# jepsen-io/maelstrom

Hardware: NVIDIA H100
Metric: simulated msgs/sec (broadcast, 4096 nodes) (higher is better)
Workload: dtype int64

## Files before the change

### maelstrom_b200/csrc/ms_device.cuh

```cuda
#pragma once
#include <stdint.h>
#include "../../include/maelstrom_b200.h"

#if defined(__CUDACC__)
#define MS_HD __host__ __device__ __forceinline__
#else
#define MS_HD inline
#endif

namespace msd {

constexpr int64_t  kTickNs   = 1000000;
constexpr uint32_t kInjector = 0xFFFFFFFFu;
constexpr uint8_t  kRemoved  = 0x80;

enum : uint32_t {
  E_NONE = 0, E_RING_OVERFLOW = 1, E_WINDOW_OVERFLOW = 2, E_JOURNAL_OVERFLOW = 3,
  E_INVALID_DEST = 4, E_HISTORY = 5, E_VALUE_RANGE = 6, E_MAIL_OVERFLOW = 7,
  E_CALENDAR_OVERFLOW = 8, E_ID_RANGE = 9, E_BARRIER = 10, E_SNAPSHOT = 11,
  E_RAFT_CAPACITY = 12, E_HISTORY_RING = 13
};

#ifndef MS_CLS0_NT
#define MS_CLS0_NT 64
// ... 132 lines not shown
  uint32_t* gs_tag;
  uint32_t* gs_snap;
  uint32_t  gs_slots, gs_interval_ms;
  uint32_t  family;
  uint32_t  sv_ep[4];
  uint32_t  sv_n_keys;
  uint32_t* sv_lin_val;
  uint8_t*  sv_lin_has;
  uint32_t* sv_lww_val;
  uint8_t*  sv_lww_has;
  uint64_t* sv_scalars;
  uint32_t* sv_seq_cli;
  uint32_t* sv_seq_vidx;
  uint32_t* sv_seq_vval;
  uint8_t*  sv_seq_vhas;
  uint32_t* sv_seq_vcnt;
  uint32_t* gs_snap_sh[8];
  uint32_t* gs_tag_sh[8];
  struct RaftDev* rf_node;
  uint4*    rf_log;
  uint32_t* rf_kv_val;
  uint8_t*  rf_kv_has;
  int32_t*  rf_next;
  int32_t*  rf_match;
  int32_t*  rf_scratch;
  uint4*    rf_cb;
  uint32_t* rf_votes;
  uint4*    rf_stage;
  uint4*    rf_heap;
  unsigned long long* rf_heap_cursor;
  uint64_t* rf_ext_off;
  uint32_t* rf_ext_tag;
  uint32_t  rf_log_cap, rf_n_keys, rf_stage_cap, rf_heap_mask, rf_vote_words;
  uint32_t  rf_group;
  uint32_t  rf_gmax;
  uint32_t  rf_cb_mask;
  struct TreeDev* tt_node;
  unsigned char* tt_recs;
  uint32_t* tt_cache;
  uint4*    tt_queue;
  uint32_t  tt_per_node, tt_cache_mask;
  struct GenDev* gc;
  uint4*    gc_hist;
  uint32_t  gc_hist_mask, gc_n, gc_read_permille, gc_pad;
  int64_t   gc_interval_ns, gc_timeout_ns, gc_limit_ns, gc_quiet_ns;
  uint4*    rf_heap_sh[8];
  uint64_t* rf_ext_off_sh[8];
  uint32_t* rf_ext_tag_sh[8];
  uint32_t  kv_value_range, kv_keys_per_group;
  int64_t   kv_key_period_ns;
  struct NemDev* nem;
  uint32_t  nem_clusters, nem_group, nem_targets, nem_pad;
  int64_t   nem_interval_ns, nem_limit_ns;
};

constexpr uint32_t kRaftCallbacks = 4096;
constexpr uint32_t kRaftExt = 1024;
constexpr int64_t  kElectionTimeoutNs = 2000000000;
constexpr int64_t  kHeartbeatNs = 1000000000;
constexpr int64_t  kMinReplicationNs = 50000000;
enum : int32_t { RAFT_NASCENT = 0, RAFT_FOLLOWER = 1, RAFT_CANDIDATE = 2, RAFT_LEADER = 3 };

struct RaftDev {
  int32_t  state;
  uint32_t term;
  int32_t  voted_for, leader;
  uint32_t commit_index, last_applied;
  int64_t  election_deadline, step_down_deadline, last_replication;
  uint32_t next_msg_id, log_size, appends, n_votes, kv_size;
  uint32_t busy;
};

constexpr uint32_t kTreeQueue = 256;
struct TreeDev {
  uint32_t ptr_counter;
  uint32_t phase;
  uint32_t cur_src, cur_msg_id;
  uint64_t cur_ops;
  uint32_t root1, root2, start_counter, writes_left, write_failed, load_ptr;
  uint32_t q_head, q_tail;
  uint32_t init_src, init_msg_id;
  uint32_t init_phase;
  uint32_t gen;
  uint32_t first_write, first_write_ok, root_is_leaf;
  uint32_t pad;
  int64_t  deadline, init_deadline;
};
constexpr int64_t kPromiseTimeoutNs = 5000000000ll;

struct GenDev {
  uint32_t next_msg_id, waiting_for;
  int64_t  deadline_ns;
  int64_t  next_op_ns;
  uint32_t node;
  uint32_t ops;
  union { uint32_t bcasts;
          uint32_t key_base; };
  uint32_t phase;
  uint32_t cur_f, cur_value;
  uint32_t ordinal;
  uint32_t reader;
};
enum : uint32_t { GEN_MIX = 0, GEN_QUIET = 1, GEN_FINAL = 2, GEN_DONE = 3 };

constexpr uint32_t kSeqBuffer = 32;
constexpr uint32_t kSeqHist = kSeqBuffer + 1;
// ... 19 lines not shown
MS_HD uint64_t mulhi64(uint64_t a, uint64_t b) {
#if defined(__CUDA_ARCH__)
  return __umul64hi(a, b);
#else
  return (uint64_t)(((unsigned __int128)a * b) >> 64);
#endif
}

MS_HD int clz64(uint64_t x) {
#if defined(__CUDA_ARCH__)
  return __clzll((long long)x);
#else
  return __builtin_clzll(x);
#endif
}

MS_HD uint64_t neg_log2_q32(uint64_t X) {
  if (X == ~0ull) return 0;
  const uint64_t Y = X + 1;
  const int n = 63 - clz64(Y);
  uint64_t m = Y << (63 - n);
  uint32_t frac = 0;
  for (int i = 31; i >= 0; i--) {
    const uint64_t hi = mulhi64(m, m);
    if (hi >> 63) { frac |= (1u << i); m = hi; }
    else          { m = hi << 1; }
  }
  return (64ull << 32) - (((uint64_t)n << 32) | frac);
}

MS_HD uint64_t latency_ms(const NetParams& np, const uint32_t x[4]) {
  if (np.dist == MS_DIST_CONSTANT) return (uint64_t)np.mean_ms * np.scale;
  if (np.dist == MS_DIST_UNIFORM)
    return (((uint64_t)x[1] * (2ull * np.mean_ms)) >> 32) * np.scale;
  const uint64_t X = ((uint64_t)x[2] << 32) | x[1];
  return mulhi64(neg_log2_q32(X), np.exp_coeff);
}

MS_HD bool kind_is_client(uint8_t k) { k &= 0x7F; return k == MS_KIND_CLIENT || k == MS_KIND_SIM_CLIENT || k == MS_KIND_GEN_CLIENT; }

MS_HD uint32_t owner_of(uint32_t e, uint32_t n_servers, uint32_t G) {
  if (G <= 1) return 0;
  if (e < n_servers) return (uint32_t)(((uint64_t)e * G) / n_servers);
  return (e - n_servers) % G;
}
MS_HD uint32_t owner_of_ticket(uint32_t t, uint32_t n_inj, uint32_t n_servers, uint32_t G) {
  return t < n_inj ? 0u : owner_of(t - n_inj, n_servers, G);
}

MS_HD uint64_t compact_round(uint64_t round, uint32_t round_lo) {
  return round - (uint32_t)((uint32_t)round - round_lo);
}

}
```

### maelstrom_b200/csrc/ms_engine.cu

```cuda
#include <cuda_runtime.h>
#include <math.h>
#include <stdio.h>
#include <stdlib.h>
#include <string.h>

#include <algorithm>
#include <deque>
#include <mutex>
#include <new>
#include <string>
#include <unordered_map>
#include <vector>

#include "ms_device.cuh"
#include "ms_nemesis.h"
#include "ms_tree.h"
#include "ms_fressian.h"
#include "ms_json.h"

using namespace msd;

extern "C" {
cudaError_t msk_round_smem_attr(size_t bytes);
size_t msk_round_smem_bytes(uint32_t cap);
// ... 541 lines not shown
  c.server_max_window = c.server_max_window ? pow2_at_least(c.server_max_window) : std::min(c.max_window, c.server_ring_cap);
  if (c.server_max_window > c.server_ring_cap) c.server_max_window = c.server_ring_cap;
  if (c.server_max_window > c.max_window) {
    set_err("server_max_window must not exceed max_window");
    return MS_ERR_ARG;
  }
  if (!c.journal_cap_log2) c.journal_cap_log2 = 22;
  if (c.journal_level > 2) c.journal_level = 2;
  if (!c.mailbox_cap) c.mailbox_cap = 1u << 16;
  if (!c.inject_cap) c.inject_cap = 1u << 16;
  if (!c.gset_interval_ms) c.gset_interval_ms = 5000;
  s->use_calendar = c.latency_mean_ms > 0;
  if (s->use_calendar) {
    c.calendar_slots = pow2_at_least(c.calendar_slots ? c.calendar_slots
                                                      : std::min<uint32_t>(16384u, std::max<uint32_t>(64u, 32u * c.latency_mean_ms)));
    const uint32_t hist = history_rows(c.reserved[0], c.max_endpoints + 8u);
    while (c.calendar_slots > 4 && c.calendar_slots > hist / 4) c.calendar_slots >>= 1;
    if (!c.calendar_cap) c.calendar_cap = 1u << 16;
  }
  if (c.n_shards == 0) c.n_shards = 1;
  if (c.n_shards > 8 || c.shard_id >= c.n_shards) { set_err("n_shards must be <= 8 and shard_id < n_shards"); return MS_ERR_ARG; }
  if (c.threads_per_node && (c.threads_per_node % 32 || c.threads_per_node > 512)) {
    set_err("threads_per_node must be a multiple of 32 in [32,512]");
    return MS_ERR_ARG;
  }
  {
    const uint32_t* ladder = kClsLadder;
    const int thr_gset[4] = {256, 256, 256, 512};
    const int* thr = c.workload == MS_W_GSET ? thr_gset : kClsThreads;
    s->n_classes = 0;
    for (int k = 0; k < 4; k++) {
      const uint32_t cap = std::min(ladder[k], c.max_window);
      s->class_cap[s->n_classes] = cap;
      s->class_threads[s->n_classes] = c.threads_per_node ? (int)c.threads_per_node : thr[k];
      s->n_classes++;
      if (cap == c.max_window) break;
    }
  }

  int ndev = 0;
  if (cudaGetDeviceCount(&ndev) != cudaSuccess || ndev == 0) {
    set_err("no CUDA device: maelstrom_b200 has no CPU fallback");
    return MS_ERR_CUDA;
  }
  s->device = c.device;
  CK(cudaSetDevice(s->device));
  CK(cudaStreamCreateWithFlags(&s->stream, cudaStreamNonBlocking));
  for (int k = 0; k < 4; k++) CK(cudaStreamCreateWithFlags(&s->aux_streams[k], cudaStreamNonBlocking));
  for (int k = 0; k < 5; k++) CK(cudaEventCreateWithFlags(&s->aux_events[k], cudaEventDisableTiming));

  Params& P = s->P;
  memset(&P, 0, sizeof P);
  const uint32_t M = c.max_endpoints;
  const bool compact = c.workload == MS_W_BROADCAST;
  const size_t n_ctr = (size_t)M + (compact ? c.n_nodes : 0u);
  int rc;
  if ((rc = s->dalloc(&P.st, 1))) return rc;
  if ((rc = s->dalloc(&P.np, 1))) return rc;
  if ((rc = s->dalloc(&P.kind, M))) return rc;
  if ((rc = s->dalloc(&P.tail, n_ctr))) return rc;
  if ((rc = s->dalloc(&P.limit, n_ctr))) return rc;
  if ((rc = s->dalloc(&P.head, n_ctr))) return rc;
  if ((rc = s->dalloc(&P.ep_born, M))) return rc;
  {
    const size_t full_vecs = ((size_t)c.n_nodes * c.server_ring_cap + (size_t)(M - c.n_nodes) * c.ring_cap) * 3;
    const size_t compact_vecs = compact ? (size_t)c.n_nodes * c.server_ring_cap : 0;
    void* ptr = nullptr;
    CK(cudaMalloc(&ptr, (full_vecs + compact_vecs) * 16));
    s->allocs.push_back(ptr);
    P.ring = (uint4*)ptr;
    P.cring_off = full_vecs;
    P.cq = compact ? M : 0u;
  }
  P.ring_cap = c.ring_cap;
  P.ring_cap_s = c.server_ring_cap;
  P.n_servers = c.n_nodes;
  P.n_ep = c.n_nodes;
  P.n_inj_tickets = 8;
  P.max_window = c.max_window;
  P.max_window_s = c.server_max_window;
  s->use_graph = c.reserved[1] == 1;
  P.n_shards = c.n_shards;
  P.shard_id = c.shard_id;
  {
    P.t_max = M + P.n_inj_tickets;
    const uint32_t hist = history_rows(c.reserved[0], P.t_max);
    P.hist = hist;
    P.hist_mask = hist - 1;
    if ((rc = s->dalloc(&P.rmeta, hist))) return rc;
    if ((rc = s->dalloc(&P.rt_em, (size_t)hist * P.t_max))) return rc;
    if ((rc = s->dalloc(&P.rt_ev, (size_t)hist * P.t_max))) return rc;
    if ((rc = s->dalloc(&P.rt_chunk, (size_t)hist * P.t_max))) return rc;
    if ((rc = s->dalloc(&P.rt_cnt, (size_t)hist * P.t_max))) return rc;
    std::vector<RoundMeta> init(hist);
    memset(init.data(), 0, init.size() * sizeof(RoundMeta));
    for (uint32_t i = 1; i < hist; i++) init[i].round = ~0ull;
    CK(cudaMemcpyAsync(P.rmeta, init.data(), init.size() * sizeof(RoundMeta), cudaMemcpyHostToDevice, s->stream));
    CK(cudaStreamSynchronize(s->stream));
  }
  P.jlevel = c.journal_level;
  P.jdiscard = c.journal_discard;
  if (c.journal_level) {
    const uint64_t J = 1ull << c.journal_cap_log2;
    void* ptr = nullptr;
    CK(cudaMalloc(&ptr, J * 16));
    s->allocs.push_back(ptr);
    P.jraw = (uint4*)ptr;
    P.jmask = J - 1;
    if (c.journal_level >= 2) {
      CK(cudaMalloc(&ptr, J * 32));
      s->allocs.push_back(ptr);
      P.jbody = (uint4*)ptr;
    }
  }
  if ((rc = s->dalloc(&P.comp, M))) return rc;
  P.seed_lo = c.seed_lo;
  P.seed_hi = c.seed_hi;
  P.workload = c.workload;
  P.topology = c.topology;
  P.n_values = c.n_values;
  P.bm_words = (c.n_values + 31) / 32;
  if (c.workload == MS_W_BROADCAST || c.workload == MS_W_GSET) {
    if ((rc = s->dalloc(&P.bitmap, (size_t)c.n_nodes * P.bm_words))) return rc;
    if ((rc = s->dalloc(&P.set_count, c.n_nodes))) return rc;
    if (c.topology != MS_TOPO_TOTAL) {
      std::vector<uint32_t> off(c.n_nodes + 1, 0), nbr, tmp;
      for (uint32_t k = 0; k < c.n_nodes; k++) {
        topo_neighbors(c.topology, c.n_nodes, k, tmp);
        nbr.insert(nbr.end(), tmp.begin(), tmp.end());
        off[k + 1] = (uint32_t)nbr.size();
      }
      if ((rc = s->dalloc(&P.nbr_off, off.size()))) return rc;
      if ((rc = s->dalloc(&P.nbr, nbr.size() + 1))) return rc;
      CK(cudaMemcpyAsync(P.nbr_off, off.data(), off.size() * 4, cudaMemcpyHostToDevice, s->stream));
      if (!nbr.empty()) CK(cudaMemcpyAsync(P.nbr, nbr.data(), nbr.size() * 4, cudaMemcpyHostToDevice, s->stream));
      CK(cudaStreamSynchronize(s->stream));
    }
  } else if (c.workload == MS_W_ECHO) {
    if ((rc = s->dalloc(&P.next_msg_id, c.n_nodes))) return rc;
  }
  P.family = c.workload == MS_W_GSET ? 1u : (c.workload >= MS_W_RAFT ? 4u : 0u);
  if (c.workload == MS_W_TXN_TREE) {
    if (c.n_shards > 1) { set_err("MS_W_TXN_TREE runs on one GPU (tree records are read across nodes)"); return MS_ERR_ARG; }
    const size_t N = c.n_nodes;
    P.tt_per_node = c.reserved[3] ? c.reserved[3] : 256u;
    P.tt_cache_mask = pow2_at_least(c.reserved[4] ? c.reserved[4] : 1024u) - 1u;
    const uint64_t n_ptrs = 2ull + (uint64_t)N * P.tt_per_node;
    if (n_ptrs > (1ull << 31)) { set_err("MS_W_TXN_TREE: n_nodes x reserved[3] pointers do not fit"); return MS_ERR_ARG; }
    if (!c.reserved[2]) c.reserved[2] = (uint32_t)n_ptrs;
    if ((rc = s->dalloc(&P.tt_node, N)) || (rc = s->dalloc(&P.tt_recs, (size_t)n_ptrs * 64)) ||
        (rc = s->dalloc(&P.tt_cache, N * ((size_t)P.tt_cache_mask + 1))) || (rc = s->dalloc(&P.tt_queue, N * kTreeQueue)))
      return rc;
    mst::Rec empty{};
    empty.type = 1; empty.lo = 0; empty.hi = (uint8_t)mst::kRing; empty.n = 0;
    CK(cudaMemcpyAsync(P.tt_recs + (size_t)(mst::kPtrEmpty - 1u) * 64, &empty, sizeof empty, cudaMemcpyHostToDevice, s->stream));
    CK(cudaStreamSynchronize(s->stream));
  }
  if (c.workload == MS_W_TXN || c.workload == MS_W_TXN_TREE) {
    const size_t N = c.n_nodes;
    P.rf_stage_cap = c.workload == MS_W_TXN_TREE ? c.server_max_window * (mst::kMaxWrites + 2u) + 64u : c.server_max_window + 16u;
    P.rf_cb_mask = pow2_at_least(c.reserved[5] ? c.reserved[5] : kRaftCallbacks) - 1u;
    if (c.workload == MS_W_TXN_TREE && P.rf_cb_mask + 1u < 128u) P.rf_cb_mask = 127u;
    if ((rc = s->dalloc(&P.rf_node, N)) || (rc = s->dalloc(&P.rf_cb, N * ((size_t)P.rf_cb_mask + 1) * 2)) ||
        (rc = s->dalloc(&P.rf_stage, N * P.rf_stage_cap * 3)))
      return rc;
  }
  if (c.workload == MS_W_RAFT) {
    const size_t N = c.n_nodes;
    P.rf_n_keys = c.reserved[2] ? c.reserved[2] : 4096u;
    P.rf_log_cap = c.reserved[3] ? c.reserved[3] : 4096u;
    P.rf_group = (c.reserved[4] && c.reserved[4] < c.n_nodes) ? c.reserved[4] : 0u;
    P.rf_gmax = P.rf_group ? P.rf_group : c.n_nodes;
    P.rf_cb_mask = pow2_at_least(c.reserved[5] ? c.reserved[5] : kRaftCallbacks) - 1u;
    P.rf_stage_cap = c.server_max_window + 2u * P.rf_gmax + P.rf_log_cap + 16u;
    P.rf_vote_words = (P.rf_gmax + 31u) / 32u;
    const uint64_t heap_want = std::max<uint64_t>(std::max<uint64_t>(1u << 16, 8ull * P.rf_log_cap), 64ull * c.n_nodes);
    if (heap_want > (1ull << 30)) { set_err("Raft payload heap too large"); return MS_ERR_ARG; }
    const uint32_t heap_words = pow2_at_least((uint32_t)heap_want);
    P.rf_heap_mask = heap_words - 1u;
    if ((rc = s->dalloc(&P.rf_node, N)) || (rc = s->dalloc(&P.rf_log, N * P.rf_log_cap * 2)) ||
        (rc = s->dalloc(&P.rf_kv_val, N * P.rf_n_keys)) || (rc = s->dalloc(&P.rf_kv_has, N * P.rf_n_keys)) ||
        (rc = s->dalloc(&P.rf_next, N * P.rf_gmax)) || (rc = s->dalloc(&P.rf_match, N * P.rf_gmax)) ||
        (rc = s->dalloc(&P.rf_scratch, N * P.rf_gmax)) || (rc = s->dalloc(&P.rf_cb, N * ((size_t)P.rf_cb_mask + 1) * 2)) ||
        (rc = s->dalloc(&P.rf_votes, N * P.rf_vote_words)) || (rc = s->dalloc(&P.rf_stage, N * P.rf_stage_cap * 3)) ||
        (rc = s->dalloc(&P.rf_heap, (size_t)heap_words)) || (rc = s->dalloc(&P.rf_heap_cursor, 1)) ||
        (rc = s->dalloc(&P.rf_ext_off, N * kRaftExt + (N * kRaftExt + 1) / 2)))
      return rc;
    P.rf_ext_tag = reinterpret_cast<uint32_t*>(P.rf_ext_off + N * kRaftExt);
// ... 1421 lines not shown
```

### maelstrom_b200/csrc/ms_kernels.cu

```cuda
#include <cuda_runtime.h>
#include <stdint.h>
#include "ms_device.cuh"
#include "ms_nemesis.h"

namespace msd {

#define FULL 0xFFFFFFFFu
#ifndef MS_EMUL
#define MS_LAUNCH(kern, grid, block, smem, stream, ...) kern<<<(grid), (block), (smem), (stream)>>>(__VA_ARGS__)
#endif
constexpr int MAXB = 64;
constexpr int MAXNB = 8;
constexpr uint64_t RECV_BIT = 1ull << 63;
constexpr uint32_t kResolvedTicket = 0xFFFFFFu;

__device__ __forceinline__ void st_v4(uint4* p, uint4 v) {
#ifdef MS_EMUL
  *p = v;
#else
  asm volatile("st.global.L1::no_allocate.v4.u32 [%0], {%1,%2,%3,%4};" ::"l"(p), "r"(v.x), "r"(v.y),
               "r"(v.z), "r"(v.w)
               : "memory");
#endif
}
// ... 17 lines not shown
  (void)gptr; (void)bytes;
#endif
}

__device__ __forceinline__ void latch_error(DevState* st, uint32_t code, uint32_t arg) {
  if (atomicCAS(&st->error, 0u, code) == 0u) st->error_arg = arg;
}

__device__ __forceinline__ bool round_skipped(const Params& p, const DevState* st) {
  if (st->now >= st->stop_ns || st->error) return true;
  if (p.jlevel && !p.jdiscard) {
    const uint64_t raw_base = p.rmeta[(uint32_t)st->round & p.hist_mask].raw_base;
    if (p.n_shards <= 1 && raw_base - st->jraw_drained > ((p.jmask + 1) >> 1)) return true;
    if (st->round - st->drain_round + 2 >= p.hist) return true;
  }
  return false;
}

__device__ __forceinline__ uint32_t slot_tag(uint64_t round) { return 0x80000000u | (uint32_t)(round & 0x7FFFFFFFull); }

struct Rec {
  uint64_t round;
  uint32_t ticket, idx;
  uint32_t src, dest, msg_id, in_reply_to;
  uint32_t tf;
  uint32_t p0;
  uint64_t p1;
};

__device__ __forceinline__ void rec_store(uint4* slot, const Rec& r) {
  st_v4(slot + 0, make_uint4(r.idx, r.ticket, (uint32_t)r.round, (uint32_t)(r.round >> 32)));
  st_v4(slot + 1, make_uint4(r.src, r.dest, r.msg_id, r.in_reply_to));
  st_v4(slot + 2, make_uint4(r.tf, r.p0, (uint32_t)r.p1, (uint32_t)(r.p1 >> 32)));
}
__device__ __forceinline__ Rec rec_unpack(uint4 a, uint4 b, uint4 c) {
  Rec r;
  r.idx = a.x; r.ticket = a.y;
  r.round = (uint64_t)a.z | ((uint64_t)a.w << 32);
  r.src = b.x; r.dest = b.y; r.msg_id = b.z; r.in_reply_to = b.w;
  r.tf = c.x; r.p0 = c.y;
  r.p1 = (uint64_t)c.z | ((uint64_t)c.w << 32);
  return r;
}

__device__ __forceinline__ uint32_t ring_cap_of(const Params& p, uint32_t e) { return e < p.n_servers ? p.ring_cap_s : p.ring_cap; }
__device__ __forceinline__ size_t ring_base(const Params& p, uint32_t e) {
  return e < p.n_servers ? (size_t)e * p.ring_cap_s
                         : (size_t)p.n_servers * p.ring_cap_s + (size_t)(e - p.n_servers) * p.ring_cap;
}
__device__ __forceinline__ uint4* ring_slot(const Params& p, uint4* ring, uint32_t e, uint32_t pos) {
  return ring + (ring_base(p, e) + (pos & (ring_cap_of(p, e) - 1u))) * 3;
}

__device__ __forceinline__ uint4* cring_slot(const Params& p, uint4* ring, uint32_t e, uint32_t pos) {
  return ring + p.cring_off + (size_t)e * p.ring_cap_s + (pos & (p.ring_cap_s - 1u));
}

struct Win {
  const uint4* ring;
  const uint4* cring;
  uint32_t head, chead, mask, n_full;
};
__device__ __forceinline__ void win_load(const Params& p, const Win& w, uint32_t e, uint64_t round, uint32_t i,
                                         uint4& a, uint4& b, uint4& c) {
  if (i < w.n_full) {
    const uint4* rp = w.ring + (size_t)((w.head + i) & w.mask) * 3;
    a = rp[0]; b = rp[1]; c = rp[2];
  } else {
    const uint4 x = w.cring[(w.chead + (i - w.n_full)) & w.mask];
    a = make_uint4(x.x, x.y, x.z, (uint32_t)(compact_round(round, x.z) >> 32));
    b = make_uint4(x.y - p.n_inj_tickets, e, 0u, 0u);
    c = make_uint4((uint32_t)MS_T_BROADCAST, x.w, 0u, 0u);
  }
}
__device__ __forceinline__ Rec win_rec(const Params& p, const Win& w, uint32_t e, uint64_t round, uint32_t i) {
  uint4 a, b, c;
  win_load(p, w, e, round, i, a, b, c);
  return rec_unpack(a, b, c);
}

struct RoundSmem {
  uint64_t* reg1;
  uint32_t* keyB;
  uint32_t* vals;
  uint16_t* tab;
  uint16_t* meta;
  uint16_t* ord;
  uint8_t* blk;
};

__device__ __forceinline__ uint64_t dense_base(const Params& p, DevState* st, uint64_t round, uint32_t ticket) {
  if (ticket == kResolvedTicket) return round << 32;
  const uint32_t row = (uint32_t)round & p.hist_mask;
  const RoundMeta* m = p.rmeta + row;
  if (m->round != round || ticket >= p.t_max) {
    latch_error(st, E_HISTORY, (uint32_t)round);
    return 0;
  }
  return m->id_base + p.rt_em[(size_t)row * p.t_max + ticket];
}

__device__ __forceinline__ uint64_t cta_excl_scan_u64(uint64_t sum, int nt, int lane, int warp, uint64_t* wtmp ) {
  uint64_t incl = sum;
#pragma unroll
  for (int d = 1; d < 32; d <<= 1) {
    const uint64_t y = __shfl_up_sync(FULL, incl, d);
    if (lane >= d) incl += y;
  }
  if (lane == 31) wtmp[warp] = incl;
  __syncthreads();
  if (warp == 0) {
    const int nw = nt >> 5;
    const uint64_t w = lane < nw ? wtmp[lane] : 0;
    uint64_t wi = w;
#pragma unroll
    for (int d = 1; d < 32; d <<= 1) {
      const uint64_t y = __shfl_up_sync(FULL, wi, d);
      if (lane >= d) wi += y;
    }
    wtmp[lane] = wi - w;
    if (lane == 31) wtmp[32] = wi;
  }
  __syncthreads();
  return wtmp[warp] + incl - sum;
}
// ... 1268 lines not shown
    if (cdirty) { p.sv_lin_has[ck] = chas ? 1 : 0; p.sv_lin_val[ck] = cval; }
  }
  __syncthreads();
}

#ifndef MS_ROUND_MINB2
#define MS_ROUND_MINB2 4
#endif
template <int CLS> struct ClsShape {
  static constexpr uint32_t cap = kClsLadder[CLS < 3 ? CLS : 2];
  static constexpr int nt = kClsThreads[CLS];
};

template <int CLS, int WL, bool FIX = false>
__global__ void __launch_bounds__(CLS == 3 ? 512 : 256, CLS == 3 ? 2 : MS_ROUND_MINB2) k_round(Params p, uint32_t cap_arg) {
  constexpr uint32_t cls = CLS;
  static_assert(!FIX || CLS < 3, "class 3 is sized by max_window");
  const uint32_t cap = FIX ? ClsShape<CLS>::cap : cap_arg;
  constexpr bool GS = (WL & 1) != 0;
  constexpr bool SV = (WL & 2) != 0;
  constexpr bool RF = (WL & 4) != 0;
  DevState* st = p.st;

#ifdef MS_EMUL
  unsigned char* smem_raw = simt::dyn_smem();
#else
  extern __shared__ __align__(16) unsigned char smem_raw[];
#endif
  uint64_t* reg1 = reinterpret_cast<uint64_t*>(smem_raw);
  uint32_t* keyB = reinterpret_cast<uint32_t*>(reg1 + cap + 1);
  uint32_t* vals = keyB + cap;
  uint16_t* tab = reinterpret_cast<uint16_t*>(vals + cap);
  uint16_t* meta = tab + 2 * (size_t)cap;
  uint16_t* ord = meta + cap;
  uint8_t* blk = reinterpret_cast<uint8_t*>(ord + cap);
  const RoundSmem sm{reg1, keyB, vals, tab, meta, ord, blk};
  uint64_t* keyA = reg1;
  uint64_t* aux = reg1;

  __shared__ uint64_t s_wtmp[34];
  __shared__ NetParams s_np;
  __shared__ uint32_t s_wcnt[17];
  __shared__ uint32_t s_misc[8];
  __shared__ uint32_t s_cnt[8];
  __shared__ uint64_t s_chunk;
  __shared__ uint16_t s_bstart[MAXB + 1];
  __shared__ uint16_t s_brank[MAXB];
  __shared__ uint16_t s_boff[MAXB + 1];
  __shared__ uint64_t s_bkeyA[MAXB];
  __shared__ uint64_t s_bbase[MAXB];
  __shared__ uint16_t s_S[MAXB + 1][MAXNB];
  __shared__ uint32_t s_nbbase[MAXNB];
  __shared__ uint32_t s_nbr[MAXNB];
  __shared__ uint4 s_gen[2];
  __shared__ uint64_t s_round0;
  __shared__ int64_t s_now0;
  __shared__ uint32_t s_go;

  const int tid = threadIdx.x, nt = FIX ? ClsShape<CLS>::nt : (int)blockDim.x, lane = tid & 31;
  if (tid == 0) {
    s_np = *p.np;
    const uint32_t so = ld_volatile_u32(&st->slot_open);
    __threadfence();
    const uint64_t r = *reinterpret_cast<const volatile uint64_t*>(&st->round);
    s_round0 = r;
    s_now0 = *reinterpret_cast<const volatile int64_t*>(&st->now);
    s_go = (so == slot_tag(r) && !round_skipped(p, st)) ? 1u : 0u;
  }
  __syncthreads();
  if (!s_go) return;
  const NetParams np = s_np;
  const int64_t now = s_now0;
  const uint64_t round = s_round0;
  const uint32_t T = p.n_inj_tickets + p.n_ep;
  const uint32_t row = (uint32_t)round & p.hist_mask;
  const uint32_t par = (uint32_t)round & 1u;
  const uint32_t my_big = st->cls_count[par][cls];
  const uint32_t my_count = my_big + st->cls_small[par][cls];
  const uint32_t* my_list = p.cls_list + ((size_t)par * 4 + cls) * p.t_max;
  const uint32_t tag = ((uint32_t)round & 0x7FFFu) + 1u;
  const bool need_rng = np.loss_thresh != 0 || np.dist != MS_DIST_CONSTANT;
  const uint64_t const_lat = (uint64_t)np.mean_ms * np.scale;
#ifdef MS_PHASE_TIMING
  const bool timing = p.phase_cycles != nullptr;
#else
  constexpr bool timing = false;
#endif
  long long t_prev = timing ? clock64() : 0;
#define PHASE_MARK(k)                                                                         \
  do {                                                                                        \
    if (timing && tid == 0) {                                                                 \
      const long long t_now = clock64();                                                      \
      atomicAdd((unsigned long long*)&p.phase_cycles[cls * 16 + (k)], (unsigned long long)(t_now - t_prev)); \
      t_prev = t_now;                                                                         \
    }                                                                                         \
  } while (0)
  if (tid == 0) s_misc[5] = atomicAdd(&st->cls_cursor[par][cls], 1u);

 for (;;) {
  __syncthreads();
  const uint32_t li = s_misc[5];
  if (tid < 5) s_misc[tid] = 0;
  if (tid < 8) s_cnt[tid] = 0;
  __syncthreads();
  if (li >= my_count) break;
  uint32_t next_li = 0;
// ... 16 lines not shown
  uint32_t c_recv_cl = 0, c_replies = 0;
  uint32_t n_ev_local = 0, n_em_local = 0;

  if (ticket < p.n_inj_tickets) {
    const uint32_t n_host = st->inj_count;
    const uint64_t tick = (uint64_t)(now / kTickNs);
    const uint32_t cur = st->sched_cursor;
    uint32_t hi = (tick + 1 < p.n_tick_off) ? p.tick_off[tick + 1] : p.n_sched;
    if (hi < cur) hi = cur;
    const uint32_t K = n_host + (hi - cur);
    const uint32_t chunk = (K + p.n_inj_tickets - 1) / p.n_inj_tickets;
    const uint32_t lo = min(ticket * chunk, K), hi_s = min(lo + chunk, K);
    const uint32_t n_local = hi_s - lo;
    n_ev_local = n_local; n_em_local = n_local;
    if (tid == 0) journal_claim(p, st, n_local, ticket, s_chunk);
    __syncthreads();
    cx.chunk = s_chunk;
    cx.emitter = kInjector;
    cx.idx_bias = lo;
    for (uint32_t base = 0; base < n_local; base += nt) {
      const uint32_t j = base + tid;
      const bool valid = j < n_local;
      Rec r;
      r.dest = 0; r.src = 0;
      if (valid) {
        const uint32_t g = lo + j;
        if (g < n_host) {
          const ms_msg m = p.inj_buf[g];
          r.src = m.src; r.dest = m.dest; r.msg_id = m.msg_id; r.in_reply_to = m.in_reply_to;
          r.tf = (uint32_t)m.type | ((uint32_t)m.flags << 16); r.p0 = m.p0; r.p1 = m.p1;
        } else {
          const ms_op op = p.sched[cur + (g - n_host)];
          r.src = op.src; r.dest = op.dest; r.msg_id = op.body.msg_id; r.in_reply_to = op.body.in_reply_to;
          r.tf = (uint32_t)op.body.type | ((uint32_t)op.body.flags << 16); r.p0 = op.body.p0; r.p1 = op.body.p1;
        }
      }
      emit_one(p, st, np, cx, valid, r, j, 0, false);
    }
  } else {
    const uint32_t e = ticket - p.n_inj_tickets;
    const uint8_t kind = p.kind[e];
    const uint32_t head = p.head[e];
    const bool has_c = p.cq && e < p.n_servers;
    const uint32_t chead = has_c ? p.head[p.cq + e] : 0u;
    uint32_t n_full = p.limit[e] - head;
    uint32_t n = n_full + (has_c ? p.limit[p.cq + e] - chead : 0u);
    if (kind & kRemoved) n = n_full = 0;
    if (n > cap || n > (e < p.n_servers ? p.max_window_s : p.max_window)) {
      if (tid == 0) latch_error(st, E_WINDOW_OVERFLOW, e);
      n = n_full = 0;
    }
    const uint4* myring = p.ring + ring_base(p, e) * 3;
    const uint32_t my_mask = ring_cap_of(p, e) - 1u;
    const Win win{myring, p.ring + p.cring_off + (size_t)e * p.ring_cap_s, head, chead, my_mask, n_full};
    const bool is_server = (kind == MS_KIND_SERVER);
    const bool bcast = !GS && is_server && p.workload == MS_W_BROADCAST;
    uint32_t n_timer = 0, fire_seq = 0, fire_p0 = 0;
    if constexpr (GS) {
      if (is_server && p.gs_init[e] && now >= p.gs_next_fire[e]) {
        n_timer = p.n_servers - 1;
        fire_seq = p.gs_fires[e] + 1;
      }
    }
    const uint32_t* mybits = (is_server && p.bitmap) ? p.bitmap + (size_t)e * p.bm_words : nullptr;
    const uint32_t deg = bcast ? nbr_count(p, e) : 0;
    const bool nb_smem = bcast && p.topology != MS_TOPO_TOTAL && deg <= MAXNB;
    if (nb_smem && tid < (int)deg) s_nbr[tid] = p.nbr[p.nbr_off[e] + tid];
    __syncthreads();

    {
      uint32_t err_val = 0xFFFFFFFFu;
      uint32_t snap_gone = 0xFFFFFFFFu;
      bool inj_srv = false;
      const bool nb4 = nb_smem && deg <= 4;
      const uint32_t nr0 = (nb4 && deg > 0) ? s_nbr[0] : 0xFFFFFFFFu, nr1 = (nb4 && deg > 1) ? s_nbr[1] : 0xFFFFFFFFu;
      const uint32_t nr2 = (nb4 && deg > 2) ? s_nbr[2] : 0xFFFFFFFFu, nr3 = (nb4 && deg > 3) ? s_nbr[3] : 0xFFFFFFFFu;
      for (int base = 0; base < (int)n; base += 2 * nt) {
        uint4 a[2], b[2], c[2];
#pragma unroll
        for (int q = 0; q < 2; q++) {
          const int i = base + q * nt + tid;
          if (i < (int)n) win_load(p, win, e, round, (uint32_t)i, a[q], b[q], c[q]);
        }
#pragma unroll
        for (int q = 0; q < 2; q++) {
          const int i = base + q * nt + tid;
          if (i >= (int)n) continue;
          const uint64_t rnd = (uint64_t)a[q].z | ((uint64_t)a[q].w << 32);
          keyA[i] = (rnd << 24) | (uint64_t)(a[q].y & 0xFFFFFFu);
          keyB[i] = a[q].x;
          const uint32_t src = b[q].x, tf = c[q].x, v = c[q].y;
          if (a[q].y < p.n_inj_tickets && src < p.n_servers) inj_srv = true;
          bool cut = false;
          if (np.pair_active && p.pair_bits)
            cut = (p.pair_bits[(size_t)e * p.pair_words + (src >> 5)] >> (src & 31)) & 1u;
          if (!cut && np.comp_active) {
            const uint32_t cs = p.comp[src], ce = p.comp[e];
            cut = cs != ce && cs != 0xFFFFFFFFu && ce != 0xFFFFFFFFu;
          }
          const uint32_t type = tf & 0xFFFFu;
          const uint32_t fl = tf >> 16;
          uint32_t tc = TC_OTHER;
          if constexpr (GS) {
            if (type == MS_T_INIT) tc = GT_INIT;
            else if (type == MS_T_ADD) tc = GT_ADD;
            else if (type == MS_T_READ) tc = GT_READ;
            else if (type == MS_T_REPLICATE_ONE) tc = GT_REPL_ONE;
            else if (type == MS_T_REPLICATE_FULL) tc = GT_REPL_FULL;
          } else {
          if (type == MS_T_INIT) tc = TC_INIT;
          else if (type == MS_T_TOPOLOGY) tc = TC_TOPOLOGY;
          else if (type == MS_T_READ) tc = TC_READ;
          else if (type == MS_T_BROADCAST) tc = TC_BROADCAST;
          else if (type == MS_T_ECHO) tc = TC_ECHO;
          }
          uint32_t slot = 0;
          if (nb4) {
            slot = src == nr3 ? 4u : src == nr2 ? 3u : src == nr1 ? 2u : src == nr0 ? 1u : 0u;
          } else if (nb_smem) {
            for (uint32_t j = 0; j < deg; j++) if (s_nbr[j] == src) slot = j + 1;
// ... 10 lines not shown
          if constexpr (GS) {
            if (is_server && !cut && !(fl & MS_F_REPLY)) {
              if (tc == GT_ADD || tc == GT_REPL_ONE) {
                if (v >= p.n_values || v > V_MASK) err_val = v;
                else val |= v;
              } else if (tc == GT_REPL_FULL) {
                const uint32_t run = c[q].z;
                const uint32_t rowi = src * p.gs_slots + (run & (p.gs_slots - 1));
                if (src >= p.n_servers ||
                    __ldcg(p.gs_tag_sh[owner_of(src, p.n_servers, p.n_shards)] + rowi) != run) snap_gone = src;
                else val |= rowi;
              }
            }
          }
          vals[i] = val;
        }
      }
      if (err_val != 0xFFFFFFFFu) latch_error(st, E_VALUE_RANGE, err_val);
      if (snap_gone != 0xFFFFFFFFu) latch_error(st, E_SNAPSHOT, snap_gone);
      if (inj_srv) s_misc[3] = 1;
    }
    if (bcast) {
      for (int base = 0; base < (int)n; base += 4 * nt) {
        uint32_t w[4], vv[4];
#pragma unroll
        for (int q = 0; q < 4; q++) {
          const int i = base + q * nt + tid;
          vv[q] = i < (int)n ? vals[i] : 0u;
          w[q] = (vv[q] & V_CAND) ? mybits[(vv[q] & V_MASK) >> 5] : 0xFFFFFFFFu;
        }
#pragma unroll
        for (int q = 0; q < 4; q++) {
          const int i = base + q * nt + tid;
          if (i < (int)n && (vv[q] & V_CAND) && !((w[q] >> (vv[q] & 31)) & 1u)) vals[i] = vv[q] | V_FRESH;
        }
      }
    }
    __syncthreads();
    PHASE_MARK(1);
    if (tid == 0 && next_li < my_count) {
      const uint32_t t2 = list_ticket(my_list, my_big, p.t_max, next_li);
      if (t2 >= p.n_inj_tickets) {
        const uint32_t e2 = t2 - p.n_inj_tickets;
        const uint32_t h2 = p.head[e2], n2 = p.limit[e2] - h2, cap2 = ring_cap_of(p, e2);
        if (n2 > 0 && n2 <= cap2) {
          const uint4* base2 = p.ring + ring_base(p, e2) * 3;
          const uint32_t o2 = h2 & (cap2 - 1u), first = min(n2, cap2 - o2);
          prefetch_l2_bulk(base2 + (size_t)o2 * 3, first * 48u);
          if (n2 > first) prefetch_l2_bulk(base2, (n2 - first) * 48u);
        }
        if (p.cq && e2 < p.n_servers) {
          const uint32_t ch2 = p.head[p.cq + e2], nc2 = p.limit[p.cq + e2] - ch2;
          if (nc2 > 0 && nc2 <= cap2) {
            const uint4* cbase2 = p.ring + p.cring_off + (size_t)e2 * cap2;
            const uint32_t o2 = ch2 & (cap2 - 1u), first = min(nc2, cap2 - o2);
            prefetch_l2_bulk(cbase2 + o2, first * 16u);
            if (nc2 > first) prefetch_l2_bulk(cbase2, (nc2 - first) * 16u);
          }
        }
      }
    }

    uint32_t R = 0;
    bool use_blocks = false;
    if (n > 0) {
      const int c = ((int)n + nt - 1) / nt;
      const int nfull = (int)n_full;
      const int lo = min(tid * c, (int)n), hi = min(lo + c, (int)n);
      uint32_t nf = 0;
      uint32_t fmask = 0;
      const bool use_mask = c <= 32;
      if (lo < hi) {
        uint64_t pa = lo ? keyA[lo - 1] : 0ull;
        uint32_t pb = lo ? keyB[lo - 1] : 0u;
        for (int i = lo; i < hi; i++) {
          const uint64_t ka = keyA[i];
          const uint32_t kb = keyB[i];
          if (i == 0 || i == nfull || ka != pa || kb <= pb) { nf++; fmask |= 1u << ((i - lo) & 31); }
          pa = ka; pb = kb;
        }
      }
      uint32_t off = block_excl_scan_v(nf, &R, s_wcnt);
      if (R <= MAXB) {
        if (use_mask) {
          while (fmask) { s_bstart[off++] = (uint16_t)(lo + __ffs(fmask) - 1); fmask &= fmask - 1u; }
        } else {
          for (int i = lo; i < hi; i++)
            if (i == 0 || i == nfull || keyA[i] != keyA[i - 1] || keyB[i] <= keyB[i - 1]) s_bstart[off++] = (uint16_t)i;
        }
        if (tid == 0) s_bstart[R] = (uint16_t)n;
        __syncthreads();
        for (uint32_t b = tid; b < R; b += nt) {
          const uint32_t s0 = s_bstart[b];
          const uint64_t ka = keyA[s0];
          const uint32_t kb = keyB[s0];
          uint32_t rk = 0;
          for (uint32_t q = 0; q < R; q++) {
            const uint32_t sq = s_bstart[q];
            const uint64_t qa = keyA[sq];
            const uint32_t qb = keyB[sq];
            if (qa < ka || (qa == ka && (qb < kb || (qb == kb && q < b)))) rk++;
          }
          s_brank[b] = (uint16_t)rk;
          s_bkeyA[rk] = ka;
          s_boff[rk] = (uint16_t)(s_bstart[b + 1] - s0);
          s_bbase[rk] = ((uint64_t)kb << 32) | keyB[s_bstart[b + 1] - 1];
        }
        __syncthreads();
        if (tid == 0) {
          uint32_t acc = 0;
// ... 303 lines not shown
    const uint32_t set_before = (is_server && p.set_count) ? p.set_count[e] : 0;
    NbrList L;
    L.nl = nb_smem ? s_nbr : nullptr;
    L.deg = deg;
    PHASE_MARK(5);

    const bool full_recv = p.jlevel >= 2 || mailed || !use_blocks;
    for (uint32_t pos = tid; pos < n; pos += nt) {
      const uint32_t i = ord[pos];
      const uint32_t val = vals[i];
      if (!(val & V_RECV)) continue;
      const uint32_t k = (uint32_t)(aux[pos] >> 32) & 0xFFFFu;
      const uint32_t mt = meta[i];
      const uint32_t sslot = mt & M_SRCSLOT;
      if (full_recv || !nb_smem || sslot == 0) {
        Rec m = win_rec(p, win, e, round, i);
        const uint64_t id = (use_blocks ? s_bbase[blk[pos]] : dense_base(p, st, m.round, m.ticket)) + m.idx;
        journal_raw(p, cx.chunk + k, id, true, m);
        const bool cl = cl_ep || (m.src >= p.n_servers && kind_is_client(p.kind[m.src]));
        if (cl) c_recv_cl++;
        if (kind == MS_KIND_SIM_CLIENT && ((m.tf >> 16) & MS_F_REPLY)) c_replies++;
        if (mailed) {
          const uint32_t mpos = s_misc[0] + k;
          if (mpos >= p.mail_cap) {
            latch_error(st, E_MAIL_OVERFLOW, e);
          } else {
            uint4* dst = reinterpret_cast<uint4*>(p.mail) + (size_t)mpos * 3;
            st_v4(dst + 0, make_uint4((uint32_t)id, (uint32_t)(id >> 32), (uint32_t)now, (uint32_t)((uint64_t)now >> 32)));
            st_v4(dst + 1, make_uint4(m.src, m.dest, m.msg_id, m.in_reply_to));
            st_v4(dst + 2, make_uint4(m.tf, m.p0, (uint32_t)m.p1, (uint32_t)(m.p1 >> 32)));
          }
        }
      } else {
        const uint64_t id = s_bbase[blk[pos]] + keyB[i];
        const uint64_t vrec = id | RECV_BIT;
        if (p.jlevel)
          st_v4(p.jraw + ((cx.chunk + k) & p.jmask),
                make_uint4((uint32_t)vrec, (uint32_t)(vrec >> 32), s_nbr[sslot - 1], e));
      }
    }
    const bool own_map = agg_mode != 2 && n_emit_msgs <= 2u * cap;
    if (own_map) {
      for (uint32_t pos = tid; pos < n; pos += nt) {
        const uint32_t e0 = (uint32_t)aux[pos], e1 = (uint32_t)aux[pos + 1];
        for (uint32_t q = e0; q < e1; q++) tab[q] = (uint16_t)pos;
      }
      __syncthreads();
    }
    for (uint32_t base = 0; base < n_emit; base += nt) {
      const uint32_t j = base + tid;
      const bool valid = j < n_emit;
      Rec r;
      r.dest = 0; r.src = e;
      uint32_t direct = 0;
      bool has_direct = false;
      bool fast = false;
      bool timer_emission = false;
      if constexpr (GS) {
        if (valid && j < n_timer) {
          timer_emission = true;
          r.dest = j < e ? j : j + 1;
          r.msg_id = 0; r.in_reply_to = 0; r.tf = MS_T_REPLICATE_FULL; r.p0 = fire_p0; r.p1 = fire_seq;
        }
      }
      if constexpr (RF) {
        if (is_server && valid && j < n_timer) {
          timer_emission = true;
          const uint4* at = p.rf_stage + ((size_t)e * p.rf_stage_cap + j) * 3;
          const uint4 a = at[0], b = at[1];
          r.src = a.x; r.dest = a.y; r.msg_id = a.z; r.in_reply_to = a.w;
          r.tf = b.x; r.p0 = b.y; r.p1 = (uint64_t)b.z | ((uint64_t)b.w << 32);
        }
      }
      if (kind == MS_KIND_GEN_CLIENT && valid && j < n_timer) {
        timer_emission = true;
        const uint4 a = s_gen[0], b = s_gen[1];
        r.src = a.x; r.dest = a.y; r.msg_id = a.z; r.in_reply_to = a.w;
        r.tf = b.x; r.p0 = b.y; r.p1 = 0;
        if constexpr (RF) r.p1 = (uint64_t)b.z | ((uint64_t)b.w << 32);
      }
      if (valid && !timer_emission) {
        const uint32_t jm = j - n_timer;
        uint32_t pos;
        if (own_map) {
          pos = tab[jm];
        } else {
          uint32_t lo = 0, hi = n;
          while (hi - lo > 1) { const uint32_t mid = (lo + hi) >> 1; if ((uint32_t)aux[mid] <= jm) lo = mid; else hi = mid; }
          pos = lo;
        }
        const uint64_t a0 = aux[pos];
        const uint32_t k = jm - (uint32_t)a0;
        const uint32_t my_emit = (uint32_t)aux[pos + 1] - (uint32_t)a0;
        const uint32_t new_before = (uint32_t)(a0 >> 48);
        const uint32_t i = ord[pos];
        const uint32_t val = vals[i];
        const uint32_t mt = meta[i];
        const bool gossip = bcast && ((mt >> M_TC_SHIFT) & 7u) == TC_BROADCAST && !(mt & M_REPLY) &&
                            !((mt & M_HAS_ID) && k == my_emit - 1);
        if (gossip && nb_smem) {
          const uint32_t ss = mt & M_SRCSLOT;
          const uint32_t js = (ss && k >= ss - 1) ? k + 1 : k;
          r.dest = s_nbr[js];
          r.msg_id = 0; r.in_reply_to = 0; r.tf = MS_T_BROADCAST; r.p0 = val & V_MASK; r.p1 = 0;
          if (agg_mode == 1) {
            direct = s_nbbase[js] + new_before - s_S[blk[pos]][js];
            has_direct = true;
          } else if (agg_mode == 2) {
            const uint32_t f = js < 2 ? (F01[pos] >> (16 * js)) : (F23[pos] >> (16 * (js - 2)));
            direct = s_nbbase[js] + new_before - (f & 0xFFFFu);
            has_direct = true;
          }
          fast = compact;
        } else {
          uint4 va, vb, vc;
          win_load(p, win, e, round, i, va, vb, vc);
          MsgView w;
          w.src = vb.x; w.msg_id = vb.z; w.tf = vc.x; w.p0 = vc.y;
          const uint64_t p1 = (uint64_t)vc.z | ((uint64_t)vc.w << 32);
          bool svc_emission = false;
          if constexpr (SV) {
            if (kind == MS_KIND_SERVICE) {
              svc_emission = true;
              r.src = e; r.dest = w.src; r.msg_id = 0; r.in_reply_to = w.msg_id;
              r.tf = (val & 0xFFFFu) | ((uint32_t)MS_F_REPLY << 16);
              r.p0 = (val >> 16) & 0xFFu;
              r.p1 = keyB[pos];
            }
          }
          if (svc_emission) {
          } else if constexpr (GS) {
            const uint32_t tc = (mt >> M_TC_SHIFT) & 7u;
            r.src = e; r.dest = w.src; r.msg_id = 0; r.in_reply_to = w.msg_id; r.p0 = 0; r.p1 = 0;
            uint32_t otype = MS_T_ERROR;
            if (tc == GT_INIT) otype = MS_T_INIT_OK;
            else if (tc == GT_ADD) otype = MS_T_ADD_OK;
            else if (tc == GT_READ) { otype = MS_T_READ_OK; r.p0 = keyB[pos]; }
            else r.p0 = 10;
            r.tf = otype | ((uint32_t)MS_F_REPLY << 16);
          } else {
          (void)node_emit(p, e, w, k, my_emit, jm, msg_id_base, set_before, new_before, p1, r, L);
          }
        }
      }
      if (fast) {
        r.round = round; r.ticket = ticket; r.idx = j;
        journal_raw(p, cx.chunk + n_recv + j, j, false, r);
        uint4* ring_o = p.ring_sh[owner_of(r.dest, p.n_servers, p.n_shards)];
        st_v4(cring_slot(p, ring_o, r.dest, direct), make_uint4(j, ticket, (uint32_t)round, r.p0));
      }
      if (__any_sync(FULL, valid && !fast)) emit_one(p, st, np, cx, valid && !fast, r, j, direct, has_direct);
    }
    if (tid == 0 && is_server) {
      if (p.workload == MS_W_ECHO && p.next_msg_id && n_emit) p.next_msg_id[e] = msg_id_base + n_emit;
      if constexpr (!GS) {
      if (p.set_count && n_new) p.set_count[e] = set_before + n_new;
      } else {
        int64_t nf = p.gs_next_fire[e];
        if (n_timer) {
          nf += (int64_t)p.gs_interval_ms * kTickNs;
          p.gs_fires[e] = fire_seq;
          p.gs_tag[e * p.gs_slots + (fire_seq & (p.gs_slots - 1))] = fire_seq;
        }
        if (s_misc[2]) { p.gs_init[e] = 1; nf = now; }
        p.gs_next_fire[e] = nf;
      }
      if (n > st->max_window_seen) atomicMax(&st->max_window_seen, n);
    }
  }

  PHASE_MARK(6);
  {
    uint32_t cnt[6] = {cx.c_send_cl, cx.c_send_sv, c_recv_cl, cx.c_lost, cx.c_zero, c_replies};
    constexpr int at[6] = {0, 1, 2, 4, 5, 7};
    if (__any_sync(FULL, (cnt[0] | cnt[1] | cnt[2] | cnt[3] | cnt[4] | cnt[5]) != 0)) {
#pragma unroll
      for (int q = 0; q < 6; q++) {
#pragma unroll
        for (int d = 16; d > 0; d >>= 1) cnt[q] += __shfl_xor_sync(FULL, cnt[q], d);
        if (lane == 0 && cnt[q]) atomicAdd(&s_cnt[at[q]], cnt[q]);
      }
      if (lane == 0 && cnt[2]) atomicAdd(&s_cnt[3], 0u - cnt[2]);
    }
  }
  __syncthreads();
  if (tid < 8 && s_cnt[tid]) {
    const uint32_t v = s_cnt[tid];
    if (tid == 0) atomicAdd((unsigned long long*)&st->stats[2], (unsigned long long)v);
    else if (tid == 1) atomicAdd((unsigned long long*)&st->stats[4], (unsigned long long)v);
    else if (tid == 2) atomicAdd((unsigned long long*)&st->stats[3], (unsigned long long)v);
    else if (tid == 3) atomicAdd((unsigned long long*)&st->stats[5], (unsigned long long)v);
    else if (tid == 4) atomicAdd((unsigned long long*)&st->lost, (unsigned long long)v);
    else if (tid == 6) atomicAdd((unsigned long long*)&st->part_drops, (unsigned long long)v);
    else if (tid == 7) atomicAdd((unsigned long long*)&st->client_replies, (unsigned long long)v);
  }
  if (tid == 0) {
    if (n_ev_local >= (1u << 23) || n_em_local >= (1u << 24)) latch_error(st, E_ID_RANGE, ticket);
    p.rt_chunk[(size_t)row * p.t_max + ticket] = cx.chunk;
    const uint64_t entry = ((uint64_t)tag << 48) | (s_cnt[5] ? (1ull << 47) : 0ull) |
                           ((uint64_t)(n_ev_local & 0x7FFFFFu) << 24) | (uint64_t)(n_em_local & 0xFFFFFFu);
    __stcg(reinterpret_cast<unsigned long long*>(p.rt_cnt + (size_t)row * p.t_max + ticket),
           (unsigned long long)entry);
// ... 379 lines not shown
```

Before: 11.84 billion.

## Shrink compact broadcast ring records to 8 bytes using reverse-neighbor slot indices

Compact ring records drop from 16 to 8 bytes. Each record now holds a 24-bit index, a 3-bit sender slot into the receiver's neighbor list, and the value. The sender's ticket and the round are rebuilt on the receiver from its shared-memory neighbor table and round-1. A host-side reverse-neighbor table is built and uploaded, and compact mode is enabled only when every node has at most 8 neighbors and all edges are symmetric. This halves ring write and read traffic and the L2 prefetch size. The cost is an extra shared-memory table, a round-1 assumption about the send round, and the limits on index width and degree.

Result: faster. 12.70 billion, median of 6 (+7.2%).

```diff
diff --git a/maelstrom_b200/csrc/ms_device.cuh b/maelstrom_b200/csrc/ms_device.cuh
--- a/maelstrom_b200/csrc/ms_device.cuh
+++ b/maelstrom_b200/csrc/ms_device.cuh
@@ -208,6 +208,7 @@
   struct NemDev* nem;
   uint32_t  nem_clusters, nem_group, nem_targets, nem_pad;
   int64_t   nem_interval_ns, nem_limit_ns;
+  uint8_t*  nbr_rev;
 };
 
 constexpr uint32_t kRaftCallbacks = 4096;
@@ -333,4 +334,30 @@
   return round - (uint32_t)((uint32_t)round - round_lo);
 }
 
-}
+struct alignas(8) CompactRec {
+  uint32_t w0, value;
+};
+constexpr uint32_t kCompactSlots = 8;
+constexpr uint32_t kCompactIdxBits = 24;
+MS_HD CompactRec compact_pack(uint32_t idx, uint32_t slot, uint32_t value) {
+  return CompactRec{(idx & ((1u << kCompactIdxBits) - 1u)) | (slot << kCompactIdxBits), value};
+}
+MS_HD uint32_t compact_idx(CompactRec r) { return r.w0 & ((1u << kCompactIdxBits) - 1u); }
+MS_HD uint32_t compact_slot(CompactRec r) { return r.w0 >> kCompactIdxBits; }
+
+inline bool nbr_reverse(const uint32_t* off, const uint32_t* nbr, uint32_t n_nodes, uint8_t* rev) {
+  for (uint32_t e = 0; e < n_nodes; e++) {
+    if (off[e + 1] - off[e] > kCompactSlots) return false;
+    for (uint32_t k = off[e]; k < off[e + 1]; k++) {
+      const uint32_t d = nbr[k];
+      if (d >= n_nodes) return false;
+      uint32_t q = off[d];
+      while (q < off[d + 1] && nbr[q] != e) q++;
+      if (q == off[d + 1]) return false;
+      rev[k] = (uint8_t)(q - off[d]);
+    }
+  }
+  return true;
+}
+
+}
diff --git a/maelstrom_b200/csrc/ms_engine.cu b/maelstrom_b200/csrc/ms_engine.cu
--- a/maelstrom_b200/csrc/ms_engine.cu
+++ b/maelstrom_b200/csrc/ms_engine.cu
@@ -617,7 +617,19 @@
   Params& P = s->P;
   memset(&P, 0, sizeof P);
   const uint32_t M = c.max_endpoints;
-  const bool compact = c.workload == MS_W_BROADCAST;
+  std::vector<uint32_t> nb_off, nb;
+  if ((c.workload == MS_W_BROADCAST || c.workload == MS_W_GSET) && c.topology != MS_TOPO_TOTAL) {
+    std::vector<uint32_t> tmp;
+    nb_off.assign(c.n_nodes + 1, 0);
+    for (uint32_t k = 0; k < c.n_nodes; k++) {
+      topo_neighbors(c.topology, c.n_nodes, k, tmp);
+      nb.insert(nb.end(), tmp.begin(), tmp.end());
+      nb_off[k + 1] = (uint32_t)nb.size();
+    }
+  }
+  std::vector<uint8_t> rev(nb.size());
+  const bool compact = c.workload == MS_W_BROADCAST && !nb_off.empty() &&
+                       nbr_reverse(nb_off.data(), nb.data(), c.n_nodes, rev.data());
   const size_t n_ctr = (size_t)M + (compact ? c.n_nodes : 0u);
   int rc;
   if ((rc = s->dalloc(&P.st, 1))) return rc;
@@ -629,9 +641,9 @@
   if ((rc = s->dalloc(&P.ep_born, M))) return rc;
   {
     const size_t full_vecs = ((size_t)c.n_nodes * c.server_ring_cap + (size_t)(M - c.n_nodes) * c.ring_cap) * 3;
-    const size_t compact_vecs = compact ? (size_t)c.n_nodes * c.server_ring_cap : 0;
+    const size_t compact_bytes = compact ? (size_t)c.n_nodes * c.server_ring_cap * sizeof(CompactRec) : 0;
     void* ptr = nullptr;
-    CK(cudaMalloc(&ptr, (full_vecs + compact_vecs) * 16));
+    CK(cudaMalloc(&ptr, full_vecs * 16 + compact_bytes));
     s->allocs.push_back(ptr);
     P.ring = (uint4*)ptr;
     P.cring_off = full_vecs;
@@ -688,17 +700,15 @@
   if (c.workload == MS_W_BROADCAST || c.workload == MS_W_GSET) {
     if ((rc = s->dalloc(&P.bitmap, (size_t)c.n_nodes * P.bm_words))) return rc;
     if ((rc = s->dalloc(&P.set_count, c.n_nodes))) return rc;
-    if (c.topology != MS_TOPO_TOTAL) {
-      std::vector<uint32_t> off(c.n_nodes + 1, 0), nbr, tmp;
-      for (uint32_t k = 0; k < c.n_nodes; k++) {
-        topo_neighbors(c.topology, c.n_nodes, k, tmp);
-        nbr.insert(nbr.end(), tmp.begin(), tmp.end());
-        off[k + 1] = (uint32_t)nbr.size();
+    if (!nb_off.empty()) {
+      if ((rc = s->dalloc(&P.nbr_off, nb_off.size()))) return rc;
+      if ((rc = s->dalloc(&P.nbr, nb.size() + 1))) return rc;
+      CK(cudaMemcpyAsync(P.nbr_off, nb_off.data(), nb_off.size() * 4, cudaMemcpyHostToDevice, s->stream));
+      if (!nb.empty()) CK(cudaMemcpyAsync(P.nbr, nb.data(), nb.size() * 4, cudaMemcpyHostToDevice, s->stream));
+      if (compact) {
+        if ((rc = s->dalloc(&P.nbr_rev, rev.size() + 1))) return rc;
+        if (!rev.empty()) CK(cudaMemcpyAsync(P.nbr_rev, rev.data(), rev.size(), cudaMemcpyHostToDevice, s->stream));
       }
-      if ((rc = s->dalloc(&P.nbr_off, off.size()))) return rc;
-      if ((rc = s->dalloc(&P.nbr, nbr.size() + 1))) return rc;
-      CK(cudaMemcpyAsync(P.nbr_off, off.data(), off.size() * 4, cudaMemcpyHostToDevice, s->stream));
-      if (!nbr.empty()) CK(cudaMemcpyAsync(P.nbr, nbr.data(), nbr.size() * 4, cudaMemcpyHostToDevice, s->stream));
       CK(cudaStreamSynchronize(s->stream));
     }
   } else if (c.workload == MS_W_ECHO) {
diff --git a/maelstrom_b200/csrc/ms_kernels.cu b/maelstrom_b200/csrc/ms_kernels.cu
--- a/maelstrom_b200/csrc/ms_kernels.cu
+++ b/maelstrom_b200/csrc/ms_kernels.cu
@@ -93,13 +93,23 @@
   return ring + (ring_base(p, e) + (pos & (ring_cap_of(p, e) - 1u))) * 3;
 }
 
-__device__ __forceinline__ uint4* cring_slot(const Params& p, uint4* ring, uint32_t e, uint32_t pos) {
-  return ring + p.cring_off + (size_t)e * p.ring_cap_s + (pos & (p.ring_cap_s - 1u));
+__device__ __forceinline__ CompactRec* cring_base(const Params& p, uint4* ring, uint32_t e) {
+  return reinterpret_cast<CompactRec*>(ring + p.cring_off) + (size_t)e * p.ring_cap_s;
+}
+static_assert(MAXNB <= (int)kCompactSlots, "a compact record's slot indexes the receiver's s_nbr");
+
+__device__ __forceinline__ void st_crec(CompactRec* p, CompactRec v) {
+#ifdef MS_EMUL
+  *p = v;
+#else
+  asm volatile("st.global.L1::no_allocate.v2.u32 [%0], {%1,%2};" ::"l"(p), "r"(v.w0), "r"(v.value) : "memory");
+#endif
 }
 
 struct Win {
   const uint4* ring;
-  const uint4* cring;
+  const CompactRec* cring;
+  const uint32_t* nbr;
   uint32_t head, chead, mask, n_full;
 };
 __device__ __forceinline__ void win_load(const Params& p, const Win& w, uint32_t e, uint64_t round, uint32_t i,
@@ -108,10 +118,12 @@
     const uint4* rp = w.ring + (size_t)((w.head + i) & w.mask) * 3;
     a = rp[0]; b = rp[1]; c = rp[2];
   } else {
-    const uint4 x = w.cring[(w.chead + (i - w.n_full)) & w.mask];
-    a = make_uint4(x.x, x.y, x.z, (uint32_t)(compact_round(round, x.z) >> 32));
-    b = make_uint4(x.y - p.n_inj_tickets, e, 0u, 0u);
-    c = make_uint4((uint32_t)MS_T_BROADCAST, x.w, 0u, 0u);
+    const CompactRec x = w.cring[(w.chead + (i - w.n_full)) & w.mask];
+    const uint32_t src = w.nbr[compact_slot(x)];
+    const uint64_t sent = round - 1u;
+    a = make_uint4(compact_idx(x), p.n_inj_tickets + src, (uint32_t)sent, (uint32_t)(sent >> 32));
+    b = make_uint4(src, e, 0u, 0u);
+    c = make_uint4((uint32_t)MS_T_BROADCAST, x.value, 0u, 0u);
   }
 }
 __device__ __forceinline__ Rec win_rec(const Params& p, const Win& w, uint32_t e, uint64_t round, uint32_t i) {
@@ -1486,6 +1498,7 @@
   __shared__ uint16_t s_S[MAXB + 1][MAXNB];
   __shared__ uint32_t s_nbbase[MAXNB];
   __shared__ uint32_t s_nbr[MAXNB];
+  __shared__ uint8_t s_rev[MAXNB];
   __shared__ uint4 s_gen[2];
   __shared__ uint64_t s_round0;
   __shared__ int64_t s_now0;
@@ -1608,7 +1621,7 @@
     }
     const uint4* myring = p.ring + ring_base(p, e) * 3;
     const uint32_t my_mask = ring_cap_of(p, e) - 1u;
-    const Win win{myring, p.ring + p.cring_off + (size_t)e * p.ring_cap_s, head, chead, my_mask, n_full};
+    const Win win{myring, cring_base(p, p.ring, e), s_nbr, head, chead, my_mask, n_full};
     const bool is_server = (kind == MS_KIND_SERVER);
     const bool bcast = !GS && is_server && p.workload == MS_W_BROADCAST;
     uint32_t n_timer = 0, fire_seq = 0, fire_p0 = 0;
@@ -1621,7 +1634,10 @@
     const uint32_t* mybits = (is_server && p.bitmap) ? p.bitmap + (size_t)e * p.bm_words : nullptr;
     const uint32_t deg = bcast ? nbr_count(p, e) : 0;
     const bool nb_smem = bcast && p.topology != MS_TOPO_TOTAL && deg <= MAXNB;
-    if (nb_smem && tid < (int)deg) s_nbr[tid] = p.nbr[p.nbr_off[e] + tid];
+    if (nb_smem && tid < (int)deg) {
+      s_nbr[tid] = p.nbr[p.nbr_off[e] + tid];
+      if (p.cq) s_rev[tid] = p.nbr_rev[p.nbr_off[e] + tid];
+    }
     __syncthreads();
 
     {
@@ -1738,10 +1754,11 @@
         if (p.cq && e2 < p.n_servers) {
           const uint32_t ch2 = p.head[p.cq + e2], nc2 = p.limit[p.cq + e2] - ch2;
           if (nc2 > 0 && nc2 <= cap2) {
-            const uint4* cbase2 = p.ring + p.cring_off + (size_t)e2 * cap2;
+            const uintptr_t cb = reinterpret_cast<uintptr_t>(cring_base(p, p.ring, e2));
             const uint32_t o2 = ch2 & (cap2 - 1u), first = min(nc2, cap2 - o2);
-            prefetch_l2_bulk(cbase2 + o2, first * 16u);
-            if (nc2 > first) prefetch_l2_bulk(cbase2, (nc2 - first) * 16u);
+            const uintptr_t s0 = (cb + (uintptr_t)o2 * 8u) & ~(uintptr_t)15, s1 = (cb + (uintptr_t)(o2 + first) * 8u + 15u) & ~(uintptr_t)15;
+            prefetch_l2_bulk(reinterpret_cast<const void*>(s0), (uint32_t)(s1 - s0));
+            if (nc2 > first) prefetch_l2_bulk(reinterpret_cast<const void*>(cb), ((nc2 - first) * 8u + 15u) & ~15u);
           }
         }
       }
@@ -2151,7 +2168,7 @@
       const bool valid = j < n_emit;
       Rec r;
       r.dest = 0; r.src = e;
-      uint32_t direct = 0;
+      uint32_t direct = 0, rslot = 0;
       bool has_direct = false;
       bool fast = false;
       bool timer_emission = false;
@@ -2211,6 +2228,7 @@
             has_direct = true;
           }
           fast = compact;
+          if (fast) rslot = s_rev[js];
         } else {
           uint4 va, vb, vc;
           win_load(p, win, e, round, i, va, vb, vc);
@@ -2245,8 +2263,8 @@
       if (fast) {
         r.round = round; r.ticket = ticket; r.idx = j;
         journal_raw(p, cx.chunk + n_recv + j, j, false, r);
-        uint4* ring_o = p.ring_sh[owner_of(r.dest, p.n_servers, p.n_shards)];
-        st_v4(cring_slot(p, ring_o, r.dest, direct), make_uint4(j, ticket, (uint32_t)round, r.p0));
+        CompactRec* cr = cring_base(p, p.ring_sh[owner_of(r.dest, p.n_servers, p.n_shards)], r.dest);
+        st_crec(cr + (direct & (p.ring_cap_s - 1u)), compact_pack(j, rslot, r.p0));
       }
       if (__any_sync(FULL, valid && !fast)) emit_one(p, st, np, cx, valid && !fast, r, j, direct, has_direct);
     }
```
